# jchristopherson/nonlin

Hardware: AMD Instinct MI355X
Metric: LM iterations/sec on m=4096,n=256 fp64; FD-Jacobian GB/s vs HBM peak (higher is better)
Workload: dtype f64

## Files before the change

### nonlin_amd/csrc/nlh_common.h

```cpp
#pragma once
#include <hip/hip_runtime.h>
#include <stdint.h>
#include <type_traits>

#define NLH_WAVE 64

enum NlhStage : int32_t {
    ST_NEED_JAC = 0,
    ST_HAVE_JAC = 1,
    ST_NE_READY = 2,
    ST_NEED_QR = 3,
    ST_QR_READY = 4,
    ST_TRIAL_READY = 5,
    ST_TRIAL_DONE = 6,
    ST_DONE = 7,
    ST_NEED_PCHOL = 8
};

struct LmState {
    double fnorm, fnorm1, par, delta, xnorm, gnorm, pnorm;
    double temp1n;
    double tailsq;
    int32_t iter, neval, njac;
    int32_t stage;
// ... 200 lines not shown
                if (plain) {
#pragma unroll
                    for (int u = 0; u < 8; ++u) s = s + d8[u];
                } else {
#pragma unroll
                    for (int u = 0; u < 8; ++u) {
                        if (c8[u] != 1.0) s = s * c8[u];
                        s = s + d8[u];
                    }
                }
            }
            for (; i < cl; ++i) {
                const double c = av[i];
                if (c != 1.0) s = s * c;
                s = s + dd[i];
            }
            carry[1] = s;
            carry[0] = fmax(mx_in, pm[cl - 1]);
        }
        __syncthreads();
    }
    const double r = carry[0] * sqrt(1.0 + carry[1]);
    __syncthreads();
    return r;
}

template <int EMAX, typename Get>
__device__ double norm2_flang_block_wide(Get get, int len, double *cd, int cap, double *aux)
{
    static_assert(EMAX % 2 == 0, "runs are read as pairs");
    const int tid = threadIdx.x, BS = blockDim.x, lane = tid & 63, wid = tid >> 6, nw = BS >> 6;
    double *cs = cd, *dsv = cd + cap, *wmax = aux, *carry = aux + 32;
    int *flags = reinterpret_cast<int *>(aux + 40);
    __syncthreads();
    if (tid == 0) { carry[0] = 0.0; carry[1] = 0.0; }
    for (int base = 0; base < len; base += cap) {
        const int cl = min(cap, len - base);
        const int E = (cl + BS - 1) / BS, i0 = tid * E;
        double a[EMAX], lm = 0.0;
#pragma unroll
        for (int u = 0; u < EMAX; ++u) {
            a[u] = (u < E && i0 + u < cl) ? fabs(get(base + i0 + u)) : 0.0;
            lm = fmax(lm, a[u]);
        }
        double sc = lm;
#pragma unroll
        for (int off = 1; off < 64; off <<= 1) {
            const double o = __shfl_up(sc, off, 64);
            if (lane >= off) sc = fmax(sc, o);
        }
        double ex = __shfl_up(sc, 1, 64);
        if (lane == 0) ex = 0.0;
        __syncthreads();
        if (lane == 63) wmax[wid] = sc;
        __syncthreads();
        const double mx_in = carry[0];
        double prev = fmax(mx_in, ex);
        for (int w = 0; w < wid; ++w) prev = fmax(prev, wmax[w]);
        bool plain = (E == EMAX) && (i0 + EMAX <= cl);
#pragma unroll
        for (int u = 0; u < EMAX; ++u) {
            if (u < E && i0 + u < cl) {
                double c = 1.0, d = 0.0;
                if (prev == 0.0) {
                } else if (a[u] > prev) {
                    const double t = prev / a[u], tsq = t * t;
                    c = tsq; d = tsq;
                } else if (a[u] != 0.0) {
                    const double t = a[u] / prev;
                    d = t * t;
                }
                plain = plain && (c == 1.0);
                cs[i0 + u] = c;
                dsv[i0 + u] = d;
                prev = fmax(prev, a[u]);
            }
        }
        flags[tid] = plain ? 1 : 0;
        __syncthreads();
        if (tid == 0) {
            double s = carry[1];
            const int nrun = (cl + E - 1) / E;
            auto general = [&](int i, int cnt) {
                for (int u = 0; u < cnt; ++u) {
                    const double c = cs[i + u];
                    if (c != 1.0) s = s * c;
                    s = s + dsv[i + u];
                }
            };
            if (E == EMAX) {
                const int nfast = nrun & ~3;
                double d0[EMAX], d1[EMAX], d2[EMAX], d3[EMAX];
                auto loadrun = [&](double (&d)[EMAX], int r) {
                    const double2 *src = reinterpret_cast<const double2 *>(dsv + r * EMAX);
#pragma unroll
                    for (int u = 0; u < EMAX / 2; ++u) { const double2 v2 = src[u]; d[2 * u] = v2.x; d[2 * u + 1] = v2.y; }
                };
                auto adds = [&](const double (&d)[EMAX]) {
#pragma unroll
                    for (int u = 0; u < EMAX; ++u) s = s + d[u];
                };
                int r = 0;
                int4 f = make_int4(0, 0, 0, 0);
                if (nfast > 0) {
                    loadrun(d0, 0); loadrun(d1, 1); loadrun(d2, 2); loadrun(d3, 3);
                    f = *reinterpret_cast<const int4 *>(flags);
                }
                for (; r < nfast; r += 4) {
                    const int4 fn = *reinterpret_cast<const int4 *>(flags + r + 4);
                    if (f.x & f.y & f.z & f.w) {
                        adds(d0); loadrun(d0, r + 4); __builtin_amdgcn_sched_barrier(0);
                        adds(d1); loadrun(d1, r + 5); __builtin_amdgcn_sched_barrier(0);
                        adds(d2); loadrun(d2, r + 6); __builtin_amdgcn_sched_barrier(0);
                        adds(d3); loadrun(d3, r + 7); __builtin_amdgcn_sched_barrier(0);
                    } else {
                        if (f.x) adds(d0); else general(r * E, E);
                        if (f.y) adds(d1); else general((r + 1) * E, E);
                        if (f.z) adds(d2); else general((r + 2) * E, E);
                        if (f.w) adds(d3); else general((r + 3) * E, min(E, cl - (r + 3) * E));
                        loadrun(d0, r + 4); loadrun(d1, r + 5); loadrun(d2, r + 6); loadrun(d3, r + 7);
                    }
                    f = fn;
                }
                for (; r < nrun; ++r) general(r * E, min(E, cl - r * E));
            } else {
                general(0, cl);
            }
            double mx = mx_in;
            for (int w = 0; w < nw; ++w) mx = fmax(mx, wmax[w]);
            carry[1] = s;
            carry[0] = mx;
        }
    }
    __syncthreads();
    const double r = carry[0] * sqrt(1.0 + carry[1]);
    __syncthreads();
    return r;
}

__device__ __forceinline__ double nlh_wave_shr1(double t)
{
    int lo = __double2loint(t), hi = __double2hiint(t);
    lo = __builtin_amdgcn_update_dpp(lo, lo, 0x138, 0xf, 0xf, false);
    hi = __builtin_amdgcn_update_dpp(hi, hi, 0x138, 0xf, 0xf, false);
    return __hiloint2double(hi, lo);
}

__device__ __forceinline__ int nlh_chain_wave(int nwaves)
{
    const unsigned b = blockIdx.x + gridDim.x * (blockIdx.y + gridDim.y * blockIdx.z);
    return (int)((b + (b >> 3) + (b >> 8)) & (unsigned)(nwaves - 1));
}

template <int EL, int BSZ, bool REGGEN = false, typename Get>
__device__ double norm2_flang_block_lanes(Get get, int len, double *cd, double *aux)
{
    constexpr int CAP = 64 * EL, E = CAP / BSZ, TPR = EL / E;
    static_assert(CAP % BSZ == 0 && EL % E == 0 && E % 2 == 0 && EL % 16 == 0, "chunk must split evenly");
    const int tid = threadIdx.x, lane = tid & 63, wid = tid >> 6;
    constexpr int nw = BSZ / 64;
    const int cw = nlh_chain_wave(nw);
    double *dsv = cd, *wmax = aux, *carry = aux + 32;
    int *tflags = reinterpret_cast<int *>(aux + 40);
    __syncthreads();
    if (tid == 0) { carry[0] = 0.0; carry[1] = 0.0; }
    for (int base = 0; base < len; base += CAP) {
        const int cl = min(CAP, len - base);
        const int i0 = tid * E;
        double a[E], lm = 0.0;
#pragma unroll
        for (int u = 0; u < E; ++u) {
            a[u] = (i0 + u < cl) ? fabs(get(base + i0 + u)) : 0.0;
            lm = fmax(lm, a[u]);
        }
        double sc = lm;
#pragma unroll
        for (int off = 1; off < 64; off <<= 1) {
            const double o = __shfl_up(sc, off, 64);
            if (lane >= off) sc = fmax(sc, o);
        }
        double ex = __shfl_up(sc, 1, 64);
        if (lane == 0) ex = 0.0;
        __syncthreads();
        if (lane == 63) wmax[wid] = sc;
        __syncthreads();
        const double mx_in = carry[0];
        double prev = fmax(mx_in, ex);
        for (int w = 0; w < wid; ++w) prev = fmax(prev, wmax[w]);
        unsigned newmax = 0;
        double2 *ddst = reinterpret_cast<double2 *>(dsv + i0 + 2 * (i0 / EL));
#pragma unroll
        for (int u = 0; u < E; u += 2) {
            double dd[2];
#pragma unroll
            for (int h = 0; h < 2; ++h) {
                const double av = a[u + h];
                const bool gt = av > prev;
                const double t = (gt ? prev : av) / (gt ? av : prev), tsq = t * t;
                const double d = (prev == 0.0) ? 0.0 : tsq;
                if (gt && prev != 0.0 && tsq != 1.0) newmax |= 1u << (u + h);
                dd[h] = d;
                prev = fmax(prev, av);
            }
            ddst[u >> 1] = make_double2(dd[0], dd[1]);
        }
        tflags[tid] = (int)newmax;
        __syncthreads();
        if (wid == cw) {
            const int nl = (cl + EL - 1) / EL;
            double d[EL];
            const double2 *mine = reinterpret_cast<const double2 *>(dsv + lane * (EL + 2));
#pragma unroll
            for (int u = 0; u < EL / 2; ++u) { const double2 v2 = mine[u]; d[2 * u] = v2.x; d[2 * u + 1] = v2.y; }
            unsigned long long nm = 0;
#pragma unroll
            for (int k = 0; k < TPR; ++k) nm |= (unsigned long long)(unsigned)tflags[lane * TPR + k] << (k * E);
            const unsigned long long mask = __ballot(nm == 0);
            double t = carry[1];
            const int ntrip = (nl + 7) >> 3;
#pragma unroll 1
            for (int g = 0; g < ntrip; ++g) {
                const unsigned m8 = (unsigned)(mask >> (8 * g)) & 0xffu;
                if (m8 == 0xffu) {
#pragma unroll
                    for (int q = 0; q < 8; ++q) {
                        t = nlh_wave_shr1(t);
#pragma unroll
                        for (int u = 0; u < EL; ++u) t = t + d[u];
                    }
                } else {
#pragma unroll 1
                    for (int q = 0; q < 8; ++q) {
                        t = nlh_wave_shr1(t);
                        if ((m8 >> q) & 1u) {
#pragma unroll
                            for (int u = 0; u < EL; ++u) t = t + d[u];
                        } else if (REGGEN) {
#pragma unroll
                            for (int u = 0; u < EL; ++u) {
                                t = t * (((nm >> u) & 1ull) ? d[u] : 1.0);
                                t = t + d[u];
                            }
                        } else {
                            const int l = 8 * g + q;
                            const unsigned long long nml = ((unsigned long long)(unsigned)__builtin_amdgcn_readlane((int)(nm >> 32), l) << 32)
                                                           | (unsigned)__builtin_amdgcn_readlane((int)nm, l);
#pragma unroll
                            for (int qd = 0; qd < EL; qd += 16) {
                                if (((nml >> qd) & 0xffffull) == 0) {
#pragma unroll
                                    for (int u = qd; u < qd + 16; ++u) t = t + d[u];
                                } else {
#pragma unroll
                                    for (int u = qd; u < qd + 16; ++u) {
                                        t = t * (((nml >> u) & 1ull) ? d[u] : 1.0);
                                        t = t + d[u];
                                    }
                                }
                            }
                        }
                    }
                }
            }
            const int lo = __builtin_amdgcn_readlane(__double2loint(t), 8 * ntrip - 1);
            const int hi = __builtin_amdgcn_readlane(__double2hiint(t), 8 * ntrip - 1);
            double mx = mx_in;
#pragma unroll
            for (int w = 0; w < nw; ++w) mx = fmax(mx, wmax[w]);
            if (lane == 0) { carry[1] = __hiloint2double(hi, lo); carry[0] = mx; }
        }
    }
    __syncthreads();
    const double r = carry[0] * sqrt(1.0 + carry[1]);
    __syncthreads();
    return r;
}

__device__ __forceinline__ void nlh_lds_barrier() { asm volatile("s_waitcnt lgkmcnt(0)\n\ts_barrier" ::: "memory"); }

__device__ __forceinline__ bool nlh_odd_ulps(double c, double inv2ulp)
{
    const double z = c * inv2ulp;
    return z != floor(z);
}
template <int EL>
__device__ __forceinline__ double ordered_possum_wave_int(const double (&d)[EL], double s0, bool &ok)
{
    const long long sb = __double_as_longlong(s0);
    const long long es = sb >> 52;
    const double ulp = __longlong_as_double((es - 52) << 52), hu = 0.5 * ulp, inv2ulp = 0.5 / ulp;
    const double C = __longlong_as_double((es << 52) | (1ll << 51)), lim = 0.25 * __longlong_as_double(es << 52);
    double c0 = 0.0, c1 = 0.0;
    bool fine = true;
#pragma unroll
    for (int u = 0; u < EL; ++u) {
        const double x = d[u];
        fine = fine && (x <= lim);
        const double t = C + x, q = t - C, r = x - q;
        const bool tie = fabs(r) == hu;
        if (__builtin_expect(__builtin_amdgcn_ballot_w64(tie) != 0ull, 0)) {
            const double f = x - hu;
            const double a0 = tie ? f + (nlh_odd_ulps(c0 + f, inv2ulp) ? ulp : 0.0) : q;
            const double a1 = tie ? f + (nlh_odd_ulps(c1 + f, inv2ulp) ? 0.0 : ulp) : q;
            c0 = c0 + a0;
            c1 = c1 + a1;
        } else {
            c0 = c0 + q;
            c1 = c1 + q;
        }
    }
#pragma unroll
    for (int off = 1; off < 64; off <<= 1) {
        const double r0 = __shfl_down(c0, off, 64), r1 = __shfl_down(c1, off, 64);
        const double n0 = c0 + (nlh_odd_ulps(c0, inv2ulp) ? r1 : r0);
        const double n1 = c1 + (nlh_odd_ulps(c1, inv2ulp) ? r0 : r1);
        c0 = n0; c1 = n1;
    }
    const double totl = (sb & 1ll) ? c1 : c0;
    const double tot = __hiloint2double(__builtin_amdgcn_readfirstlane(__double2hiint(totl)), __builtin_amdgcn_readfirstlane(__double2loint(totl)));
    const double out = s0 + tot;
    ok = (__builtin_amdgcn_ballot_w64(!fine) == 0ull) && ((__double_as_longlong(out) >> 52) == es);
    return out;
}

template <int EL, int BSZ, typename Get>
__device__ double norm2_flang_block_lanes_pipe(Get get, int len, double *cd, double *aux, double *wm)
{
    constexpr int CAP = 64 * EL, PADCAP = CAP + 128, E = CAP / BSZ, TPR = EL / E, nw = BSZ / 64;
    static_assert(CAP % BSZ == 0 && EL % E == 0 && E % 2 == 0, "chunk must split evenly");
    const int tid = threadIdx.x, lane = tid & 63, wid = tid >> 6;
    const bool prep = wid < nw, chain = (wid == nw);
    const int nch = (len + CAP - 1) / CAP, i0 = tid * E;
    int *tflags = reinterpret_cast<int *>(aux + 8);
    auto loadabs = [&](int c, double (&a)[E]) __attribute__((always_inline)) {
        const int base = c * CAP, cl = min(CAP, len - base);
#pragma unroll
        for (int u = 0; u < E; ++u) a[u] = (i0 + u < cl) ? fabs(get(base + i0 + u)) : 0.0;
    };
    auto scanmax = [&](int c, const double (&a)[E]) __attribute__((always_inline)) {
        double lm = 0.0;
#pragma unroll
        for (int u = 0; u < E; ++u) lm = fmax(lm, a[u]);
        double sc = lm;
#pragma unroll
        for (int off = 1; off < 64; off <<= 1) {
            const double o = __shfl_up(sc, off, 64);
            if (lane >= off) sc = fmax(sc, o);
        }
        double ex = __shfl_up(sc, 1, 64);
        if (lane == 0) ex = 0.0;
        if (lane == 63) wm[c * nw + wid] = sc;
        return ex;
    };
    double a0[E], a1[E], ex0 = 0.0;
    __syncthreads();
    if (prep) {
        loadabs(0, a0);
        if (nch > 1) loadabs(1, a1);
        ex0 = scanmax(0, a0);
    }
    __syncthreads();
    double mxrun = 0.0, s = 0.0;
    for (int c = 0; c < nch; ++c) {
        const int cl = min(CAP, len - c * CAP);
        double *dsv = cd + (size_t)(c & 1) * PADCAP;
        int *tf = tflags + (c & 1) * BSZ;
        double mxc = mxrun;
#pragma unroll
        for (int w = 0; w < nw; ++w) mxc = fmax(mxc, wm[c * nw + w]);
        if (prep) {
            double prev = fmax(mxrun, ex0);
#pragma unroll
            for (int w = 0; w < nw; ++w)
                if (w < wid) prev = fmax(prev, wm[c * nw + w]);
            unsigned newmax = 0;
            double2 *ddst = reinterpret_cast<double2 *>(dsv + i0 + 2 * (i0 / EL));
#pragma unroll
            for (int u = 0; u < E; u += 2) {
                double dd[2];
#pragma unroll
                for (int h = 0; h < 2; ++h) {
                    double d = 0.0;
                    const double av = a0[u + h];
                    if (prev == 0.0) {
                    } else if (av > prev) {
                        const double t = prev / av, tsq = t * t;
                        d = tsq;
                        if (tsq != 1.0) newmax |= 1u << (u + h);
                    } else if (av != 0.0) {
                        const double t = av / prev;
                        d = t * t;
                    }
                    dd[h] = d;
                    prev = fmax(prev, av);
                }
                ddst[u >> 1] = make_double2(dd[0], dd[1]);
            }
            tf[tid] = (int)newmax;
            if (c + 1 < nch) {
#pragma unroll
                for (int u = 0; u < E; ++u) a0[u] = a1[u];
// ... 247 lines not shown
```

### nonlin_amd/csrc/nlh_qrx.hip

```cpp
#include "nlh_qrx.h"
#include "nlh_common.h"
#include "../../include/nonlin_hip.h"
#include <type_traits>
#include <cstdio>
#include <cstdlib>
#include <algorithm>

#ifndef QRX_C
#define QRX_C 10
#endif
#define QRX_TR 64
#define QRX_PAD_ROWS 160
#ifndef QRX_AUX_LOAD
#define QRX_AUX_LOAD 0
#endif
#ifndef QRX_AUX_STORE
#define QRX_AUX_STORE 1
#endif
#ifndef QRX_UF
#define QRX_UF(flush) 16
#endif

typedef unsigned int qrx_u32x2 __attribute__((ext_vector_type(2)));
typedef unsigned int qrx_u32x4 __attribute__((ext_vector_type(4)));
// ... 35 lines not shown
    auto take = [&](size_t bytes) { size_t o = off; off += (bytes + 255) & ~(size_t)255; return o; };
    const size_t oV = take(sizeof(double) * ((size_t)nprob * 2 * QRX_C * qrx_vstride(m) + 2 * QRX_TR));
    const size_t otp = take(sizeof(double) * (size_t)nprob * 2 * QRX_C * (n + 1));
    const size_t ord = take(sizeof(double) * (size_t)nprob * n);
    const size_t owa = take(sizeof(double) * (size_t)nprob * n);
    const size_t ost = take(sizeof(QrxStep) * (size_t)nprob);
    const size_t osr = take(sizeof(int32_t) * (size_t)nprob * (n + 1));
    const size_t oso = take(sizeof(int32_t) * (size_t)nprob * qrx_ld(n));
    const size_t opl = take(sizeof(int32_t) * (size_t)nprob);
    if (w) {
        char *b = (char *)base;
        w->V = (double *)(b + oV); w->tp = (double *)(b + otp); w->rdiag = (double *)(b + ord);
        w->wa = (double *)(b + owa); w->step = (QrxStep *)(b + ost); w->src = (int32_t *)(b + osr);
        w->slotof = (int32_t *)(b + oso);
        w->plist = (int32_t *)(b + opl);
    }
    return off;
}

size_t qrx_workspace_bytes(int nprob, int m, int n) { return qrx_carve(nullptr, nprob, m, n, nullptr); }

__global__ void __launch_bounds__(256)
k_qrx_transpose(int m, int n, int ld, int coff, size_t tst, const double *__restrict__ J, double *__restrict__ T,
                const LmState *__restrict__ st)
{
    const int p = blockIdx.y;
    if (st && st[p].stage != ST_NEED_QR) return;
    const double *Jp = J + (size_t)p * m * n;
    double *Tp = T + (size_t)p * tst;
    const int nblk = (m + 7) >> 3;
    const size_t total = (size_t)nblk * n;
    for (size_t e = (size_t)blockIdx.x * blockDim.x + threadIdx.x; e < total; e += (size_t)gridDim.x * blockDim.x) {
        const int k = (int)(e % n), b = (int)(e / n);
        const double *src = Jp + (size_t)k * m + (size_t)b * 8;
        double *dst = Tp + ((size_t)b * ld + coff + k) * 8;
        double vv[8];
#pragma unroll
        for (int r = 0; r < 8; ++r) vv[r] = (b * 8 + r < m) ? src[r] : 0.0;
#pragma unroll
        for (int r = 0; r < 8; ++r) dst[r] = vv[r];
    }
}

__global__ void __launch_bounds__(256)
k_qrx_list(int nprob, int ny, LmState *__restrict__ st, int32_t *__restrict__ plist)
{
    __shared__ int wsum[4], base;
    const int tid = threadIdx.x, lane = tid & 63, wid = tid >> 6;
    if (tid == 0) base = 0;
    __syncthreads();
    for (int p0 = 0; p0 < nprob; p0 += 256) {
        const int p = p0 + tid;
        const bool on = p < nprob && st[p].stage == ST_NEED_QR;
        const unsigned long long b = __ballot(on);
        const int before = __popcll(b & ((1ull << lane) - 1ull));
        if (lane == 0) wsum[wid] = __popcll(b);
        __syncthreads();
        int off = base;
        for (int w2 = 0; w2 < wid; ++w2) off += wsum[w2];
        if (on) {
            const int pos = off + before;
            if (pos < ny) plist[pos] = p;
            else { st[p].flag = 1; st[p].stage = ST_DONE; }
        }
        __syncthreads();
        if (tid == 0) base += wsum[0] + wsum[1] + wsum[2] + wsum[3];
        __syncthreads();
    }
    for (int i = base + tid; i < ny; i += 256) plist[i] = -1;
}

__global__ void __launch_bounds__(256)
k_qrx_init_norms(int m, int n, int ld, int coff, size_t tst, const double *__restrict__ T, QrxWs w, LmVecs v,
                 const LmState *__restrict__ st)
{
    __shared__ __attribute__((aligned(16))) double cd[64 * 64 + 128];
    __shared__ __attribute__((aligned(16))) double aux[40 + 128];
    const int p = w.plist ? w.plist[blockIdx.y] : (int)blockIdx.y, k = blockIdx.x;
    if (p < 0 || (st && st[p].stage != ST_NEED_QR)) return;
    const double *a = T + (size_t)p * tst;
    const double nr = norm2_flang_block_lanes<64, 256>([&](int i) { return a[qrx_at(i, coff + k, ld)]; }, m, cd, aux);
    if (threadIdx.x == 0) {
        v.acnorm[(size_t)p * n + k] = nr;
        w.rdiag[(size_t)p * n + k] = nr;
        w.wa[(size_t)p * n + k] = nr;
        v.ipvt[(size_t)p * n + k] = k;
    }
}

template <bool NORMS>
__global__ void __launch_bounds__(256)
k_qrx_init(int m, int n, int ld, int coff, size_t tst, double *__restrict__ T, const double *__restrict__ fall, QrxWs w, LmVecs v,
           const LmState *__restrict__ st)
{
    const int p = blockIdx.x;
    if (st && st[p].stage != ST_NEED_QR) return;
    const int tid = threadIdx.x, BS = blockDim.x;
    double *a = T + (size_t)p * tst;
    const double *f = fall + (size_t)p * m;
    for (int i = tid; i < m; i += BS) a[qrx_at(i, coff + n, ld)] = f[i];
    for (int k = tid; NORMS && k < n; k += BS) {
        double mx = 0.0, sq = 0.0;
        auto step = [&](double vv) {
            const double av = fabs(vv);
            if (mx == 0.0) {
                mx = av;
            } else if (av > mx) {
                const double t = mx / av, tsq = t * t;
                sq = sq * tsq;
                sq = sq + tsq;
                mx = av;
            } else if (av != 0.0) {
                const double t = av / mx;
                sq = sq + t * t;
            }
        };
        const int nblk = (m + 7) >> 3;
        const double *colp = a + (size_t)(coff + k) * 8;
        double xa[8], xb[8];
        auto ld8 = [&](double (&x)[8], int b) {
#pragma unroll
            for (int r = 0; r < 8; ++r) x[r] = colp[(size_t)b * ld * 8 + r];
        };
        ld8(xa, 0);
        for (int b = 0; b < nblk; b += 2) {
            if (b + 1 < nblk) ld8(xb, b + 1);
#pragma unroll
            for (int r = 0; r < 8; ++r) if (b * 8 + r < m) step(xa[r]);
            if (b + 2 < nblk) ld8(xa, b + 2);
            if (b + 1 < nblk) {
#pragma unroll
                for (int r = 0; r < 8; ++r) if ((b + 1) * 8 + r < m) step(xb[r]);
            }
        }
        const double nr = mx * sqrt(1.0 + sq);
        v.acnorm[(size_t)p * n + k] = nr;
        w.rdiag[(size_t)p * n + k] = nr;
        w.wa[(size_t)p * n + k] = nr;
        v.ipvt[(size_t)p * n + k] = k;
    }
    for (int k = tid; k <= n; k += BS) w.src[(size_t)p * (n + 1) + k] = coff + k;
    for (int c = tid; c < ld; c += BS) w.slotof[(size_t)p * ld + c] = c >= coff ? c - coff : -1;
}

#define QRX_LONG_EL 48
#define QRX_LONG_THREADS 256
#ifndef QRX_LONG_GU
#define QRX_LONG_GU 8
#endif
#ifndef QRX_LONG_SU
#define QRX_LONG_SU 4
#endif
#ifndef QRX_PIV64_WG
#define QRX_PIV64_WG 1
#endif
#define QRX_LONG_MAXCH 96
template <int QRX_NL, bool LONG = false, bool FEW = false>
__global__ void __launch_bounds__(LONG ? QRX_LONG_THREADS : 256, (QRX_NL == 32 && !FEW) ? 4 : (QRX_NL == 64 && !FEW && !LONG) ? QRX_PIV64_WG : 1)
k_qrx_pivot(int p0, int m, int n, int ld, int coff, size_t tst, size_t vst, int j, int cur, int np, int flush, double *__restrict__ T, QrxWs w,
            double *__restrict__ Rall, LmVecs v, const LmState *__restrict__ st)
{
    __shared__ __attribute__((aligned(16))) double cd[LONG ? 2 * (64 * QRX_LONG_EL + 128) : (64 * QRX_NL + (FEW ? 256 : 128))];
    __shared__ __attribute__((aligned(16))) double aux[LONG ? 8 + 256 : 40 + 128];
    __shared__ double wmx[LONG ? 3 * QRX_LONG_MAXCH : 1];
    __shared__ double red[64];
    const int p = p0 + blockIdx.x;
    if (st && st[p].stage != ST_NEED_QR) return;
    const int tid = threadIdx.x, BS = blockDim.x, ldp = n + 1;
#ifdef QRX_DBG_CLK
    long long clk[6]; clk[0] = wall_clock64();
#endif
    int *redi = reinterpret_cast<int *>(red + 32);
    double *rdiag = w.rdiag + (size_t)p * n, *wa = w.wa + (size_t)p * n;
    int32_t *src = w.src + (size_t)p * ldp;
    int32_t *ipvt = v.ipvt + (size_t)p * n;
    double *tpc = w.tp + ((size_t)p * 2 + cur) * QRX_C * ldp;
    double *R = Rall + (size_t)p * n * n;

    const bool onecand = (n - j <= BS);
    int32_t *slotof = w.slotof + (size_t)p * ld;
    const bool fresh = (flush & 2) != 0;
    if (fresh) {
        for (int c = tid; c < ld; c += BS) slotof[c] = (c - coff >= j && c - coff <= n) ? c - coff : -1;
        for (int k = j + tid; k <= n; k += BS) src[k] = coff + k;
    }
    double bv = 0.0, my_tk[QRX_C - 1];
    int bk = 0x7fffffff, my_src = 0, my_ipvt = 0;
    if (onecand) {
        const int k = j + tid;
        if (k < n) {
            bv = rdiag[k]; bk = k;
            my_src = fresh ? coff + k : src[k]; my_ipvt = ipvt[k];
#pragma unroll
            for (int q = 0; q < QRX_C - 1; ++q) my_tk[q] = (q < np) ? tpc[(size_t)q * ldp + k] : 0.0;
        }
    } else {
        for (int k = j + tid; k < n; k += BS) {
            const double d = rdiag[k];
            if (bk == 0x7fffffff || d > bv) { bv = d; bk = k; }
        }
    }
    double rd_j = 0.0, wa_j = 0.0;
    int src_j = 0, ipvt_j = 0, src_0 = 0;
    if (tid == 0) { rd_j = rdiag[j]; wa_j = wa[j]; src_j = fresh ? coff + j : src[j]; ipvt_j = ipvt[j]; src_0 = src[0]; }
    __shared__ uint32_t amx[3 * 16];
    const int kmax = (QRX_NL == 32 && onecand) ? j + block_argmax_first_norms(bv, bk != 0x7fffffff, amx) : block_argmax_first(bv, bk, red, redi);
    double *pub = red + 40;
    int *pubi = reinterpret_cast<int *>(pub + QRX_C);
    if (onecand) {
        if (j + tid == kmax) {
#pragma unroll
            for (int q = 0; q < QRX_C - 1; ++q) pub[q] = my_tk[q];
            pubi[0] = my_src; pubi[1] = my_ipvt;
        }
    } else if (tid == 0) {
        pubi[0] = fresh ? coff + kmax : src[kmax]; pubi[1] = ipvt[kmax];
    } else if (tid <= np) {
        pub[tid - 1] = tpc[(size_t)(tid - 1) * ldp + kmax];
    }
    __syncthreads();
    const int srck = pubi[0];
#ifdef QRX_DBG_CLK
    clk[1] = wall_clock64();
#endif
    double tk[QRX_C];
#pragma unroll
    for (int q = 0; q < QRX_C; ++q) tk[q] = (q < QRX_C - 1 && q < np) ? pub[q] : 0.0;
    if (kmax != j) {
        if (tid == 0) {
            rdiag[kmax] = rd_j;
            wa[kmax] = wa_j;
            ipvt[j] = pubi[1]; ipvt[kmax] = ipvt_j;
            if (j == 0) {
                slotof[src_0] = -1;
                slotof[srck] = kmax;
            } else {
                src[kmax] = src_j;
                slotof[src_j] = kmax;
                slotof[srck] = -1;
            }
        }
        if (tid < np) tpc[(size_t)tid * ldp + kmax] = tpc[(size_t)tid * ldp + j];
        for (int i = tid; i < j; i += BS) {
            const double t = R[(size_t)j * n + i];
            R[(size_t)j * n + i] = R[(size_t)kmax * n + i];
            R[(size_t)kmax * n + i] = t;
        }
    } else if (tid == 0) {
        slotof[srck] = -1;
    }
    const bool move0 = (j == 0 && kmax != 0);
    if (LONG && (flush & 8)) {
        if (tid == 0) {
            QrxStep s;
            s.ajnorm = 0.0; s.ajj = 0.0; s.kmax = kmax; s.srck = srck; s.t0 = np ? tk[0] : 0.0;
            w.step[p] = s;
        }
        return;
    }
    const int src0 = coff;
    const double *__restrict__ Vc = w.V + ((size_t)p * 2 + cur) * QRX_C * vst;
    double *__restrict__ Vn = (flush & 1) ? w.V + ((size_t)p * 2 + (cur ^ 1)) * QRX_C * vst
                                    : w.V + (((size_t)p * 2 + cur) * QRX_C + np) * vst;
    double *Tp = T + (size_t)p * tst;
    const bool staged = !LONG && (m - j <= 64 * QRX_NL);
    double *stage = cd;
    auto spos = [](int i) __attribute__((always_inline)) { return FEW ? i + i / (64 * QRX_NL / 256) : i; };
    constexpr int KEEP = 64 * QRX_NL / 256;
    double keep[KEEP];
#pragma unroll
    for (int u = 0; u < KEEP; ++u) keep[u] = 0.0;
    auto gather4 = [&](int i0, double (&e)[4]) __attribute__((always_inline)) {
        double vq[4][QRX_C - 1], mv[4];
#pragma unroll
        for (int u = 0; u < 4; ++u) {
            const int row = min(i0 + u * BS, m - 1);
            e[u] = Tp[qrx_at(row, srck, ld)];
            mv[u] = move0 ? Tp[qrx_at(row, src0, ld)] : 0.0;
#pragma unroll
            for (int q = 0; q < QRX_C - 1; ++q) vq[u][q] = (q < np) ? Vc[(size_t)q * vst + row] : 0.0;
        }
#pragma unroll
        for (int u = 0; u < 4; ++u) {
#pragma unroll
            for (int q = 0; q < QRX_C - 1; ++q)
                if (q < np) e[u] = e[u] - tk[q] * vq[u][q];
            if (move0 && i0 + u * BS < m) Tp[qrx_at(i0 + u * BS, srck, ld)] = mv[u];
        }
    };
    if (FEW && staged && np == 1 && !move0) {
        double e[KEEP], pv[KEEP];
#pragma unroll
        for (int u = 0; u < KEEP; ++u) {
            const int row = min(j + tid + u * BS, m - 1);
            e[u] = Tp[qrx_at(row, srck, ld)];
            pv[u] = Vc[row];
        }
#pragma unroll
        for (int u = 0; u < KEEP; ++u) { asm volatile("" : "+v"(e[u])); asm volatile("" : "+v"(pv[u])); }
#pragma unroll
        for (int u = 0; u < KEEP; ++u) {
            e[u] = e[u] - tk[0] * pv[u];
            keep[u] = e[u];
            if (j + tid + u * BS < m) stage[spos(tid + u * BS)] = e[u];
        }
    } else if (staged) {
#pragma unroll
        for (int it = 0; it < KEEP / 4; ++it) {
            const int i0 = j + tid + it * 4 * BS;
            if (i0 < m) {
                double e[4];
                gather4(i0, e);
#pragma unroll
                for (int u = 0; u < 4; ++u) {
                    keep[it * 4 + u] = e[u];
                    if (i0 + u * BS < m) stage[spos(i0 + u * BS - j)] = e[u];
                }
            }
        }
    } else if (LONG && np <= 1 && !move0) {
        const int jb = j & ~7, npair = (m - jb + 1) >> 1;
        const double *colp = Tp + qrx_at(jb, srck, ld);
        const size_t blk = (size_t)ld * 8;
        const double t0 = np ? tk[0] : 0.0;
        constexpr int GU = QRX_LONG_GU;
        for (int pb = tid; pb < npair; pb += GU * BS) {
            double2 ax[GU], px[GU];
#pragma unroll
            for (int u = 0; u < GU; ++u) {
                const int pr = min(pb + u * BS, npair - 1);
                ax[u] = *reinterpret_cast<const double2 *>(colp + (size_t)(pr >> 2) * blk + 2 * (pr & 3));
                px[u] = np ? *reinterpret_cast<const double2 *>(Vc + jb + 2 * pr) : make_double2(0.0, 0.0);
            }
#pragma unroll
            for (int u = 0; u < GU; ++u) {
                const int pr = pb + u * BS, row = jb + 2 * pr;
                if (pr >= npair) continue;
                if (np) { ax[u].x = ax[u].x - t0 * px[u].x; ax[u].y = ax[u].y - t0 * px[u].y; }
                if (row >= j && row + 1 < m) *reinterpret_cast<double2 *>(Vn + row) = ax[u];
                else {
                    if (row >= j && row < m) Vn[row] = ax[u].x;
                    if (row + 1 >= j && row + 1 < m) Vn[row + 1] = ax[u].y;
                }
            }
        }
    } else {
        for (int i0 = j + tid; i0 < m; i0 += 4 * BS) {
            double e[4];
            gather4(i0, e);
#pragma unroll
            for (int u = 0; u < 4; ++u)
                if (i0 + u * BS < m) Vn[i0 + u * BS] = e[u];
        }
    }
    __syncthreads();
    const double ejj = staged ? stage[0] : Vn[j];
#ifdef QRX_DBG_CLK
    clk[2] = wall_clock64();
#endif
    double ajnorm;
    if constexpr (LONG) ajnorm = norm2_flang_block_lanes_pipe<QRX_LONG_EL, 192>([&](int i) { return Vn[j + i]; }, m - j, cd, aux, wmx);
    else ajnorm = staged ? norm2_flang_block_lanes<QRX_NL, 256, FEW>([&](int i) { return stage[spos(i)]; }, m - j, cd, aux)
                         : norm2_flang_block_lanes<QRX_NL, 256, FEW>([&](int i) { return Vn[j + i]; }, m - j, cd, aux);
#ifdef QRX_DBG_CLK
    clk[3] = wall_clock64();
#endif
    double ajj = 0.0;
    if (staged) {
        if (ajnorm != 0.0 && ejj < 0.0) ajnorm = -ajnorm;
        const double dn = (ajnorm != 0.0) ? ajnorm : 1.0;
#pragma unroll
        for (int u = 0; u < KEEP; ++u) keep[u] = keep[u] / dn;
#pragma unroll
        for (int u = 0; u < KEEP; ++u) {
            const int i = j + tid + u * BS;
            double t = keep[u];
            if (ajnorm != 0.0 && i == j) { t = t + 1.0; ajj = t; }
            if (i < m) Vn[i] = t;
        }
    } else if (LONG && (flush & 4) && ajnorm != 0.0) {
        if (ejj < 0.0) ajnorm = -ajnorm;
        if (tid == 0) { ajj = ejj / ajnorm + 1.0; Vn[j] = ajj; }
    } else if (LONG && ajnorm != 0.0) {
        if (ejj < 0.0) ajnorm = -ajnorm;
        const int jb = j & ~7, nsec = (m - jb + 7) >> 3;
        for (int sb = tid; sb < nsec; sb += QRX_LONG_SU * BS) {
            double2 tx[QRX_LONG_SU][4];
#pragma unroll
            for (int q = 0; q < QRX_LONG_SU; ++q) {
                const double2 *sp = reinterpret_cast<const double2 *>(Vn + jb + (size_t)min(sb + q * BS, nsec - 1) * 8);
#pragma unroll
                for (int h = 0; h < 4; ++h) tx[q][h] = sp[h];
            }
#pragma unroll
            for (int q = 0; q < QRX_LONG_SU; ++q) {
                const int sc = sb + q * BS, row = jb + sc * 8;
                if (sc >= nsec) continue;
#pragma unroll
                for (int h = 0; h < 4; ++h) {
                    tx[q][h].x = tx[q][h].x / ajnorm;
                    tx[q][h].y = tx[q][h].y / ajnorm;
                    if (row + 2 * h == j) { tx[q][h].x = tx[q][h].x + 1.0; ajj = tx[q][h].x; }
                    if (row + 2 * h + 1 == j) { tx[q][h].y = tx[q][h].y + 1.0; ajj = tx[q][h].y; }
                }
                if (row >= j && row + 8 <= m) {
                    double2 *dp = reinterpret_cast<double2 *>(Vn + row);
#pragma unroll
                    for (int h = 0; h < 4; ++h) dp[h] = tx[q][h];
                } else {
#pragma unroll
                    for (int h = 0; h < 4; ++h) {
                        if (row + 2 * h >= j && row + 2 * h < m) Vn[row + 2 * h] = tx[q][h].x;
                        if (row + 2 * h + 1 >= j && row + 2 * h + 1 < m) Vn[row + 2 * h + 1] = tx[q][h].y;
                    }
                }
            }
        }
    } else if (ajnorm != 0.0) {
        if (ejj < 0.0) ajnorm = -ajnorm;
        for (int i0 = j + tid; i0 < m; i0 += 8 * BS) {
            double t[8];
#pragma unroll
            for (int u = 0; u < 8; ++u) t[u] = Vn[min(i0 + u * BS, m - 1)];
#pragma unroll
            for (int u = 0; u < 8; ++u) {
                t[u] = t[u] / ajnorm;
                if (i0 + u * BS == j) { t[u] = t[u] + 1.0; ajj = t[u]; }
                if (i0 + u * BS < m) Vn[i0 + u * BS] = t[u];
            }
        }
    }
#ifdef QRX_DBG_CLK
    clk[4] = wall_clock64();
    if (tid == 0 && j == 100) printf("pivot j=100: head %lld gather %lld norm %lld scale %lld (x10 ns)\n", clk[1]-clk[0], clk[2]-clk[1], clk[3]-clk[2], clk[4]-clk[3]);
#endif
    if (tid == 0) {
        QrxStep s;
        s.ajnorm = ajnorm; s.ajj = ajj; s.kmax = kmax; s.srck = srck; s.t0 = 0.0;
        w.step[p] = s;
        rdiag[j] = -ajnorm;
    }
}

__global__ void __launch_bounds__(256)
k_qrx_gather_long(int m, int ld, size_t tst, size_t vst, int j, int cur, int np, int flush, const double *__restrict__ T, QrxWs w,
                  const LmState *__restrict__ st)
{
    const int p = blockIdx.y;
    if (st && st[p].stage != ST_NEED_QR) return;
    const QrxStep step = w.step[p];
    const double *Tp = T + (size_t)p * tst;
    const double *__restrict__ Vc = w.V + ((size_t)p * 2 + cur) * QRX_C * vst;
    double *__restrict__ Vn = (flush & 1) ? w.V + ((size_t)p * 2 + (cur ^ 1)) * QRX_C * vst
                                    : w.V + (((size_t)p * 2 + cur) * QRX_C + np) * vst;
    const int jb = j & ~7, npair = (m - jb + 1) >> 1;
    const double *colp = Tp + qrx_at(jb, step.srck, ld);
    const size_t blk = (size_t)ld * 8;
    const double t0 = step.t0;
    const int pb = (blockIdx.x * 256 + threadIdx.x) * 4;
    double2 ax[4], px[4];
#pragma unroll
    for (int u = 0; u < 4; ++u) {
        const int pr = min(pb + u, npair - 1);
        ax[u] = *reinterpret_cast<const double2 *>(colp + (size_t)(pr >> 2) * blk + 2 * (pr & 3));
        px[u] = np ? *reinterpret_cast<const double2 *>(Vc + jb + 2 * pr) : make_double2(0.0, 0.0);
    }
#pragma unroll
    for (int u = 0; u < 4; ++u) {
        const int pr = pb + u, row = jb + 2 * pr;
        if (pr >= npair) continue;
        if (np) { ax[u].x = ax[u].x - t0 * px[u].x; ax[u].y = ax[u].y - t0 * px[u].y; }
        if (row >= j && row + 1 < m) *reinterpret_cast<double2 *>(Vn + row) = ax[u];
        else {
            if (row >= j && row < m) Vn[row] = ax[u].x;
            if (row + 1 >= j && row + 1 < m) Vn[row + 1] = ax[u].y;
        }
    }
}

#ifndef QRX_NORM_PREP
#define QRX_NORM_PREP 384
#endif
#define QRX_NORM_THREADS (QRX_NORM_PREP + 64)
__global__ void __launch_bounds__(QRX_NORM_THREADS)
k_qrx_norm_long(int m, int n, size_t vst, int j, int cur, int np, int flush, QrxWs w, const LmState *__restrict__ st)
{
    __shared__ __attribute__((aligned(16))) double cd[2 * (64 * QRX_LONG_EL + 128)];
    __shared__ __attribute__((aligned(16))) double aux[8 + QRX_NORM_PREP];
    __shared__ double wmx[(QRX_NORM_PREP / 64) * QRX_LONG_MAXCH];
    const int p = blockIdx.x;
    if (st && st[p].stage != ST_NEED_QR) return;
    double *__restrict__ Vn = (flush & 1) ? w.V + ((size_t)p * 2 + (cur ^ 1)) * QRX_C * vst
                                    : w.V + (((size_t)p * 2 + cur) * QRX_C + np) * vst;
    const double ejj = Vn[j];
    double ajnorm = norm2_flang_block_lanes_pipe<QRX_LONG_EL, QRX_NORM_PREP>([&](int i) { return Vn[j + i]; }, m - j, cd, aux, wmx);
    if (threadIdx.x == 0) {
        QrxStep s = w.step[p];
        double ajj = 0.0;
        if (ajnorm != 0.0) {
            if (ejj < 0.0) ajnorm = -ajnorm;
            ajj = ejj / ajnorm + 1.0;
            Vn[j] = ajj;
        }
        s.ajnorm = ajnorm; s.ajj = ajj;
        w.step[p] = s;
        w.rdiag[(size_t)p * n + j] = -ajnorm;
    }
}

__global__ void __launch_bounds__(256)
k_qrx_scale_long(int m, size_t vst, int j, int cur, int np, int flush, QrxWs w, const LmState *__restrict__ st)
{
    const int p = blockIdx.y;
    if (st && st[p].stage != ST_NEED_QR) return;
    const double ajnorm = w.step[p].ajnorm;
    if (ajnorm == 0.0) return;
    double *__restrict__ Vn = (flush & 1) ? w.V + ((size_t)p * 2 + (cur ^ 1)) * QRX_C * vst
                                    : w.V + (((size_t)p * 2 + cur) * QRX_C + np) * vst;
    const int first = (j + 2) & ~1;
    if (blockIdx.x == 0 && threadIdx.x == 0 && first == j + 2 && j + 1 < m) Vn[j + 1] = Vn[j + 1] / ajnorm;
    const int npair = (m - first) >> 1;
    const int pb = (blockIdx.x * 256 + threadIdx.x) * 4;
    double2 t[4];
#pragma unroll
    for (int u = 0; u < 4; ++u) t[u] = (pb + u < npair) ? *reinterpret_cast<const double2 *>(Vn + first + 2 * (pb + u)) : make_double2(0.0, 0.0);
#pragma unroll
    for (int u = 0; u < 4; ++u)
        if (pb + u < npair) {
            t[u].x = t[u].x / ajnorm; t[u].y = t[u].y / ajnorm;
            *reinterpret_cast<double2 *>(Vn + first + 2 * (pb + u)) = t[u];
        }
    if (blockIdx.x == 0 && threadIdx.x == 0 && ((m - first) & 1)) Vn[m - 1] = Vn[m - 1] / ajnorm;
}

template <int NP, bool FLUSH>
__device__ __forceinline__ void
qrx_pass_tail(int p, int j, int k, int col, int wcol, int m, int n, int ld, int cur, size_t vst, double s, double rowj, double rk, double wak,
              bool refl, double ajj, const double (&tq)[NP > 0 ? NP : 1], const double *__restrict__ Tp, const double *__restrict__ vc,
              const double *__restrict__ vo, double *__restrict__ tpall,
              double *__restrict__ rdall, double *__restrict__ waall, double *__restrict__ Rall, double *__restrict__ qtfall)
{
    constexpr int NPI = NP < QRX_C ? NP : 0;
    const int ldp = n + 1, jb = j & ~7;
    double *tpc = tpall + ((size_t)p * 2 + cur) * QRX_C * ldp;
    auto pending = [&](double a, const auto &vr) {
        double e = a;
#pragma unroll
        for (int q = 0; q < NP; ++q) e = e - tq[q] * vr[q];
        return e;
    };
    double *tpn = FLUSH ? tpall + ((size_t)p * 2 + (cur ^ 1)) * QRX_C * ldp : tpc + (size_t)NPI * ldp;
    double *rdiag = rdall + (size_t)p * n, *wa = waall + (size_t)p * n;
    const double temp = refl ? s / ajj : 0.0;
    tpn[k] = temp;
    const double rjk = refl ? rowj - temp * ajj : rowj;
    if (k == n) { qtfall[(size_t)p * n + j] = rjk; return; }
    Rall[(size_t)p * n * n + (size_t)k * n + j] = rjk;
    if (!refl) return;
    if (rk != 0.0) {
        const double t2 = rjk / rk;
        rk = rk * sqrt(fmax(0.0, 1.0 - t2 * t2));
        const double q = rk / wak;
        if (!(5.0e-2 * (q * q) > NLH_EPS)) {
            rk = norm2_flang_serial([&](int i2) {
                const int row = j + 1 + i2, rel = row - jb;
                double vr[NP + 1];
#pragma unroll
                for (int q2 = 0; q2 < NP; ++q2) vr[q2] = vc[(size_t)q2 * vst + rel];
                const double e = FLUSH ? Tp[qrx_at(row, wcol, ld)] : pending(Tp[qrx_at(row, col, ld)], vr);
                const double vn = FLUSH ? vo[rel] : vc[(size_t)NPI * vst + rel];
                return e - temp * vn;
            }, m - j - 1);
            wa[k] = rk;
        }
        rdiag[k] = rk;
    }
}

#define QRX_SHARE_MAXWIN 4
template <int NP, bool FLUSH, bool SHARE>
__global__ void __launch_bounds__(SHARE ? 64 * QRX_SHARE_MAXWIN : 64) __attribute__((amdgpu_waves_per_eu(1, (FLUSH && NP >= 4) ? 2 : 4)))
k_qrx_pass(int p0, int nprob, int nwin, int lo, int m, int n, int ld, int coff, size_t tst, size_t vst, int j, int cur,
           double *T, double *Tout, const double *__restrict__ Vall, double *__restrict__ tpall,
           int32_t *__restrict__ srcall, int32_t *__restrict__ slotall, double *__restrict__ rdall,
           double *__restrict__ waall, const QrxStep *__restrict__ stepall, double *__restrict__ Rall,
           double *__restrict__ qtfall, const LmState *__restrict__ st)
{
// ... 1246 lines not shown
```

Baseline: 3834.

## Split norm carry chain across two waves and raise pivot kernel occupancy

Adds a SPLIT mode to the block-wide Fortran-compatible norm2 reduction. For the 64-element-per-lane pivot path, each lane's run is halved and the sequential carry chain is processed by two waves in turn, with a barrier between them. This shortens per-wave register arrays and the serial dependency length per wave. It also raises the min-waves-per-EU launch bound for the 64-row pivot kernel from 1 to 3, trading registers for occupancy, and reworks debug clock printing to store timestamps per workgroup. Risks include register spills under the tighter bound and an extra sync per chunk.

```diff
diff --git a/nonlin_amd/csrc/nlh_common.h b/nonlin_amd/csrc/nlh_common.h
--- a/nonlin_amd/csrc/nlh_common.h
+++ b/nonlin_amd/csrc/nlh_common.h
@@ -376,11 +376,12 @@
     return (int)((b + (b >> 3) + (b >> 8)) & (unsigned)(nwaves - 1));
 }
 
-template <int EL, int BSZ, bool REGGEN = false, typename Get>
+template <int EL, int BSZ, bool REGGEN = false, bool SPLIT = false, typename Get>
 __device__ double norm2_flang_block_lanes(Get get, int len, double *cd, double *aux)
 {
-    constexpr int CAP = 64 * EL, E = CAP / BSZ, TPR = EL / E;
-    static_assert(CAP % BSZ == 0 && EL % E == 0 && E % 2 == 0 && EL % 16 == 0, "chunk must split evenly");
+    constexpr int CAP = 64 * EL, E = CAP / BSZ;
+    constexpr int HR = SPLIT ? EL / 2 : EL, NH = EL / HR, TPR = HR / E;
+    static_assert(CAP % BSZ == 0 && HR % E == 0 && E % 2 == 0 && HR % 16 == 0 && NH <= BSZ / 64, "chunk must split evenly");
     const int tid = threadIdx.x, lane = tid & 63, wid = tid >> 6;
     constexpr int nw = BSZ / 64;
     const int cw = nlh_chain_wave(nw);
@@ -430,15 +431,20 @@
         }
         tflags[tid] = (int)newmax;
         __syncthreads();
-        if (wid == cw) {
-            const int nl = (cl + EL - 1) / EL;
-            double d[EL];
-            const double2 *mine = reinterpret_cast<const double2 *>(dsv + lane * (EL + 2));
-#pragma unroll
-            for (int u = 0; u < EL / 2; ++u) { const double2 v2 = mine[u]; d[2 * u] = v2.x; d[2 * u + 1] = v2.y; }
+        const int nruns = (cl + HR - 1) / HR;
+#pragma unroll 1
+        for (int h = 0; h < NH && 64 * h < nruns; ++h) {
+            if (h) __syncthreads();
+            if (wid != ((cw + h) & (nw - 1))) continue;
+            const int nl = min(64, nruns - 64 * h);
+            const int e0 = (64 * h + lane) * HR;
+            double d[HR];
+            const double2 *mine = reinterpret_cast<const double2 *>(dsv + e0 + 2 * (e0 / EL));
+#pragma unroll
+            for (int u = 0; u < HR / 2; ++u) { const double2 v2 = mine[u]; d[2 * u] = v2.x; d[2 * u + 1] = v2.y; }
             unsigned long long nm = 0;
 #pragma unroll
-            for (int k = 0; k < TPR; ++k) nm |= (unsigned long long)(unsigned)tflags[lane * TPR + k] << (k * E);
+            for (int k = 0; k < TPR; ++k) nm |= (unsigned long long)(unsigned)tflags[(64 * h + lane) * TPR + k] << (k * E);
             const unsigned long long mask = __ballot(nm == 0);
             double t = carry[1];
             const int ntrip = (nl + 7) >> 3;
@@ -450,7 +456,7 @@
                     for (int q = 0; q < 8; ++q) {
                         t = nlh_wave_shr1(t);
 #pragma unroll
-                        for (int u = 0; u < EL; ++u) t = t + d[u];
+                        for (int u = 0; u < HR; ++u) t = t + d[u];
                     }
                 } else {
 #pragma unroll 1
@@ -458,10 +464,10 @@
                         t = nlh_wave_shr1(t);
                         if ((m8 >> q) & 1u) {
 #pragma unroll
-                            for (int u = 0; u < EL; ++u) t = t + d[u];
+                            for (int u = 0; u < HR; ++u) t = t + d[u];
                         } else if (REGGEN) {
 #pragma unroll
-                            for (int u = 0; u < EL; ++u) {
+                            for (int u = 0; u < HR; ++u) {
                                 t = t * (((nm >> u) & 1ull) ? d[u] : 1.0);
                                 t = t + d[u];
                             }
@@ -470,7 +476,7 @@
                             const unsigned long long nml = ((unsigned long long)(unsigned)__builtin_amdgcn_readlane((int)(nm >> 32), l) << 32)
                                                            | (unsigned)__builtin_amdgcn_readlane((int)nm, l);
 #pragma unroll
-                            for (int qd = 0; qd < EL; qd += 16) {
+                            for (int qd = 0; qd < HR; qd += 16) {
                                 if (((nml >> qd) & 0xffffull) == 0) {
 #pragma unroll
                                     for (int u = qd; u < qd + 16; ++u) t = t + d[u];
diff --git a/nonlin_amd/csrc/nlh_qrx.hip b/nonlin_amd/csrc/nlh_qrx.hip
--- a/nonlin_amd/csrc/nlh_qrx.hip
+++ b/nonlin_amd/csrc/nlh_qrx.hip
@@ -211,9 +211,12 @@
 #define QRX_LONG_SU 4
 #endif
 #ifndef QRX_PIV64_WG
-#define QRX_PIV64_WG 1
+#define QRX_PIV64_WG 3
 #endif
 #define QRX_LONG_MAXCH 96
+#ifdef QRX_DBG_CLK
+__device__ long long qrx_dbg_clk[8192][5];
+#endif
 template <int QRX_NL, bool LONG = false, bool FEW = false>
 __global__ void __launch_bounds__(LONG ? QRX_LONG_THREADS : 256, (QRX_NL == 32 && !FEW) ? 4 : (QRX_NL == 64 && !FEW && !LONG) ? QRX_PIV64_WG : 1)
 k_qrx_pivot(int p0, int m, int n, int ld, int coff, size_t tst, size_t vst, int j, int cur, int np, int flush, double *__restrict__ T, QrxWs w,
@@ -418,9 +421,10 @@
     clk[2] = wall_clock64();
 #endif
     double ajnorm;
+    constexpr bool CSPLIT = QRX_NL == 64 && !FEW;
     if constexpr (LONG) ajnorm = norm2_flang_block_lanes_pipe<QRX_LONG_EL, 192>([&](int i) { return Vn[j + i]; }, m - j, cd, aux, wmx);
-    else ajnorm = staged ? norm2_flang_block_lanes<QRX_NL, 256, FEW>([&](int i) { return stage[spos(i)]; }, m - j, cd, aux)
-                         : norm2_flang_block_lanes<QRX_NL, 256, FEW>([&](int i) { return Vn[j + i]; }, m - j, cd, aux);
+    else ajnorm = staged ? norm2_flang_block_lanes<QRX_NL, 256, FEW, CSPLIT>([&](int i) { return stage[spos(i)]; }, m - j, cd, aux)
+                         : norm2_flang_block_lanes<QRX_NL, 256, FEW, CSPLIT>([&](int i) { return Vn[j + i]; }, m - j, cd, aux);
 #ifdef QRX_DBG_CLK
     clk[3] = wall_clock64();
 #endif
@@ -491,7 +495,12 @@
     }
 #ifdef QRX_DBG_CLK
     clk[4] = wall_clock64();
-    if (tid == 0 && j == 100) printf("pivot j=100: head %lld gather %lld norm %lld scale %lld (x10 ns)\n", clk[1]-clk[0], clk[2]-clk[1], clk[3]-clk[2], clk[4]-clk[3]);
+    if (tid == 0 && j == 100 && blockIdx.x < 8192)
+        for (int q = 0; q < 5; ++q) qrx_dbg_clk[blockIdx.x][q] = clk[q];
+    if (tid == 0 && j == 101 && blockIdx.x < 8192) {
+        const long long *c = qrx_dbg_clk[blockIdx.x];
+        printf("pivot j=100 wg %d: start %lld head %lld gather %lld norm %lld scale %lld (x10 ns)\n", (int)blockIdx.x, c[0], c[1]-c[0], c[2]-c[1], c[3]-c[2], c[4]-c[3]);
+    }
 #endif
     if (tid == 0) {
         QrxStep s;
```

Result: faster. 3877 (median of 4 runs) (+1.1%).
